# JuliaSmoothOptimizers/Krylov.jl

Measured on NVIDIA H100. Metric: CG iterations/s, higher is better.
Workload: dtype f64

## Files before the change

### krylov.jl_b200/csrc/cg_fused.cu

```cuda
#include "solver_common.h"
#include "spmv_tiles.cuh"

namespace kb {

constexpr int kHist = 64;

template <class T>
struct CgState {
  T gamma, pAp, alpha, beta, pNorm2, rNorm, eps_tol, pad0;
  int iter, itmax, done, linesearch;
  int solved, tired, zero_curvature, inconsistent;
  int npc, not_spd, comm_error, pad2;
  T hist[kHist];
};

static_assert(sizeof(CgState<double>) % 8 == 0 && sizeof(CgState<float>) % 8 == 0, "CgState is copied as 8-byte words");

template <class T>
struct CgPeers {
  HaloMap halo;
  const T* r[kMaxRanks];
  const T* p_old[kMaxRanks];
  const T* mdiag;
  const T* r_halo;
  const T* p_halo_old;
  PushPlan<T> push_p;
};

template <class T>
__device__ __forceinline__ void cg_k1_finalize(CgState<T>* st, T pAp) {
  st->pAp = pAp;
  const T lim = mul_rn(Eps<T>::v, st->pNorm2);
  if (pAp <= lim) {
    if (fabs(pAp) <= lim) { st->zero_curvature = 1; st->inconsistent = !st->linesearch; }
    if (st->linesearch) { st->npc = 1; st->solved = 1; }
    if (st->zero_curvature || st->solved) { st->done = 1; return; }
  }
  st->alpha = div_rn(st->gamma, pAp);
}

template <class T>
__device__ __forceinline__ void cg_k2_finalize(CgState<T>* st, T gamma_next) {
  if (!(gamma_next >= T(0))) { st->not_spd = 1; st->done = 1; return; }
  const T rNorm = sqrt_rn(gamma_next);
  st->rNorm = rNorm;
  const int it1 = st->iter + 1;
  st->hist[it1 % kHist] = rNorm;
  const bool solved = (rNorm <= st->eps_tol) || (add_rn(rNorm, T(1)) <= T(1));
  if (!solved) {
    const T beta = div_rn(gamma_next, st->gamma);
    st->beta = beta;
    st->pNorm2 = add_rn(gamma_next, mul_rn(mul_rn(beta, beta), st->pNorm2));
    st->gamma = gamma_next;
  }
  st->iter = it1;
  st->solved = solved;
  st->tired = it1 >= st->itmax;
  st->done = solved || st->tired;
}

template <class T>
__device__ __forceinline__ bool cg_global_sum(CgState<T>* st, DistComm* dc, T& v) {
  if (dc) {
    v = dist_reduce(dc, v);
    if (dc->error) { st->comm_error = 1; st->done = 1; return false; }
  }
  return true;
}

constexpr int kPlain = 0, kDist = 1, kJacobi = 2, kBlockJac = 3;

template <class T, int MODE>
struct PVal {
  const T* r; const T* p_old; T beta; const CgPeers<T>* peers;
  const T* mdiag;
  __device__ __forceinline__ T operator()(int j) const {
    if (MODE == kDist && j >= peers->halo.nloc) {
      const int h = j - peers->halo.nloc;
      if (peers->r_halo)
        return add_rn(__ldg(&peers->r_halo[h]), mul_rn(beta, __ldg(&peers->p_halo_old[h])));
      const int rk = __ldg(&peers->halo.src_rank[h]), off = __ldg(&peers->halo.src_off[h]);
      return add_rn(__ldg(&peers->r[rk][off]), mul_rn(beta, __ldg(&peers->p_old[rk][off])));
    }
    T z = __ldg(&r[j]);
    if (MODE == kJacobi) z = mul_rn(__ldg(&mdiag[j]), z);
    return add_rn(z, mul_rn(beta, __ldg(&p_old[j])));
  }
};

template <class T> struct RowPre { T pn, po, xr; };

template <class T, int MODE, int MINB, bool XUP>
__global__ void __launch_bounds__(kTileThreads, MINB) cg_k1_tma(Csr<T> A, const T* __restrict__ r, const T* __restrict__ p_old,
                                                          T* __restrict__ p_new, T* __restrict__ Ap, CgState<T>* st,
                                                          T* part, unsigned* ticket, DistComm* dc, CgPeers<T> peers,
                                                          T* __restrict__ x) {
  extern __shared__ __align__(128) unsigned char smem[];
  __shared__ T sm[32];
  if (*(volatile int*)&st->done) return;
  T dacc = T(0);
  bool sent = false;
  const T beta = st->beta, alpha_prev = st->alpha;
  const bool xup = XUP && st->iter > 0;
  const PVal<T, MODE> pval{r, p_old, beta, &peers, peers.mdiag};
  auto row_begin = [&](int row) {
    RowPre<T> q;
    q.po = __ldg(&p_old[row]);
    T z = __ldg(&r[row]);
    if (MODE == kJacobi) z = mul_rn(__ldg(&peers.mdiag[row]), z);
    q.pn = add_rn(z, mul_rn(beta, q.po));
    q.xr = xup ? x[row] : T(0);
    return q;
  };
  spmv_tiles_run<T>(A, smem, pval, row_begin, [&](int row, T acc, RowPre<T> q) {
    p_new[row] = q.pn;
    if (MODE == kDist) sent |= peers.push_p(row, q.pn);
    Ap[row] = acc;
    if (xup) x[row] = add_rn(q.xr, mul_rn(alpha_prev, q.po));
    dacc += q.pn * acc;
  });
  if (MODE == kDist && sent) __threadfence_system();
  T mine[1] = {block_sum(dacc, sm)}, tot[1];
  if (grid_sum_last<T, 1>(mine, part, ticket, sm, tot) && threadIdx.x == 0) {
    if (cg_global_sum(st, MODE == kDist ? dc : nullptr, tot[0])) cg_k1_finalize(st, tot[0]);
  }
}

template <class T, int MODE, bool XUP>
__global__ void __launch_bounds__(kBlock) cg_k1_rows(Csr<T> A, const T* __restrict__ r, const T* __restrict__ p_old,
                                                     T* __restrict__ p_new, T* __restrict__ Ap, CgState<T>* st, T* part,
                                                     unsigned* ticket, DistComm* dc, CgPeers<T> peers, T* __restrict__ x) {
  __shared__ T sm[32];
  if (*(volatile int*)&st->done) return;
  T dacc = T(0);
  bool sent = false;
  const T alpha_prev = st->alpha;
  const bool xup = XUP && st->iter > 0;
  const PVal<T, MODE> pval{r, p_old, st->beta, &peers, peers.mdiag};
  const int stride = gridDim.x * blockDim.x;
  for (int row = blockIdx.x * blockDim.x + threadIdx.x; row < A.n; row += stride) {
    const int kb = A.rowptr[row], ke = A.rowptr[row + 1];
    T acc = T(0);
    for (int k = kb; k < ke; k++) acc = add_rn(acc, mul_rn(A.val[k], pval(A.colind[k])));
    const T pn = pval(row);
    p_new[row] = pn;
    if (MODE == kDist) sent |= peers.push_p(row, pn);
    Ap[row] = acc;
    if (xup) x[row] = add_rn(x[row], mul_rn(alpha_prev, __ldg(&p_old[row])));
    dacc += pn * acc;
  }
  if (MODE == kDist && sent) __threadfence_system();
  T mine[1] = {block_sum(dacc, sm)}, tot[1];
  if (grid_sum_last<T, 1>(mine, part, ticket, sm, tot) && threadIdx.x == 0) {
    if (cg_global_sum(st, MODE == kDist ? dc : nullptr, tot[0])) cg_k1_finalize(st, tot[0]);
  }
}

template <class T, int MODE, bool XK2>
__global__ void __launch_bounds__(kBlock) cg_k2(int n, T* __restrict__ x, T* __restrict__ r, const T* __restrict__ p,
                                                const T* __restrict__ Ap, CgState<T>* st, T* part, unsigned* ticket,
                                                DistComm* dc, const T* __restrict__ mdiag, PushPlan<T> push_r) {
  __shared__ T sm[32];
  if (*(volatile int*)&st->done) return;
  const T alpha = st->alpha, nalpha = -alpha;
  T acc = T(0);
  bool sent = false;
  const int stride = gridDim.x * blockDim.x;
  int i = blockIdx.x * blockDim.x + threadIdx.x;
  for (; i + 3 * stride < n; i += 4 * stride) {
    T xv[4], rv[4], pv[4], av[4];
#pragma unroll
    for (int u = 0; u < 4; u++) {
      const int j = i + u * stride;
      rv[u] = r[j]; av[u] = __ldg(&Ap[j]);
      if (XK2) { xv[u] = x[j]; pv[u] = __ldg(&p[j]); }
    }
#pragma unroll
    for (int u = 0; u < 4; u++) {
      const int j = i + u * stride;
      if (XK2) x[j] = add_rn(xv[u], mul_rn(alpha, pv[u]));
      const T rn = add_rn(rv[u], mul_rn(nalpha, av[u]));
      r[j] = rn;
      if (MODE == kDist) sent |= push_r(j, rn);
      acc += rn * (MODE == kJacobi ? mul_rn(__ldg(&mdiag[j]), rn) : rn);
    }
  }
  for (; i < n; i += stride) {
    const int j = i;
    if (XK2) x[j] = add_rn(x[j], mul_rn(alpha, p[j]));
    const T rn = add_rn(r[j], mul_rn(nalpha, Ap[j]));
    r[j] = rn;
    if (MODE == kDist) sent |= push_r(j, rn);
    acc += rn * (MODE == kJacobi ? mul_rn(__ldg(&mdiag[j]), rn) : rn);
  }
  if (MODE == kDist && sent) __threadfence_system();
  T mine[1] = {block_sum(acc, sm)}, tot[1];
  if (grid_sum_last<T, 1>(mine, part, ticket, sm, tot) && threadIdx.x == 0) {
    if (cg_global_sum(st, dc, tot[0])) cg_k2_finalize(st, tot[0]);
  }
}

struct GridBar { unsigned count, gen, halo_ready, timed_iters; unsigned long long ns_a, ns_b; };

__device__ __forceinline__ unsigned ld_acquire_gpu_u32(const unsigned* p) {
  unsigned v;
  asm volatile("ld.acquire.gpu.global.u32 %0, [%1];" : "=r"(v) : "l"(p) : "memory");
  return v;
}
__device__ __forceinline__ void st_release_gpu_u32(unsigned* p, unsigned v) {
  asm volatile("st.release.gpu.global.u32 [%0], %1;" ::"l"(p), "r"(v) : "memory");
}
__device__ __forceinline__ double ld_sys(const double* p) {
  double v;
  asm volatile("ld.relaxed.sys.global.f64 %0, [%1];" : "=d"(v) : "l"(p) : "memory");
  return v;
}
__device__ __forceinline__ float ld_sys(const float* p) {
  float v;
  asm volatile("ld.relaxed.sys.global.f32 %0, [%1];" : "=f"(v) : "l"(p) : "memory");
  return v;
}

template <class T> struct CgScal { T alpha, beta; int iter, done; };
template <class T>
__device__ __forceinline__ void cg_load_scal(const CgState<T>* st, CgScal<T>* sc) {
  const volatile CgState<T>* v = st;
  const T al = v->alpha, be = v->beta;
  const int it = v->iter, dn = v->done;
  sc->alpha = al; sc->beta = be; sc->iter = it; sc->done = dn;
}

template <class T, class Fin>
__device__ __forceinline__ bool grid_reduce_barrier(GridBar* gb, T v, T* part, T* sm, unsigned* sflag, const CgState<T>* st,
                                                    CgScal<T>* sc, Fin fin) {
  const T mine = block_sum(v, sm);
  if (threadIdx.x == 0) {
    const unsigned g = *(volatile unsigned*)&gb->gen;
    __stcg(&part[blockIdx.x], mine);
    __threadfence();
    const unsigned t = atomicAdd(&gb->count, 1u);
    sflag[0] = (t == gridDim.x - 1);
    sflag[1] = g;
  }
  __syncthreads();
  const bool last = sflag[0] != 0;
  const unsigned g = sflag[1];
  bool ok = true;
  if (last) {
    if (threadIdx.x < 32) {
      __threadfence();
      T acc = T(0);
      for (int i = threadIdx.x; i < (int)gridDim.x; i += 32) acc += __ldcg(&part[i]);
      const T tot = warp_sum(acc);
      fin(tot);
      __syncwarp();
      if (threadIdx.x == 0) {
        cg_load_scal<T>(st, sc);
        gb->count = 0u;
        st_release_gpu_u32(&gb->gen, g + 1u);
      }
    }
  } else if (threadIdx.x == 0) {
    const long long t0 = clock64();
    while (ld_acquire_gpu_u32(&gb->gen) == g) {
      if (clock64() - t0 > 120000000000LL) { sflag[0] = 2; break; }
    }
    cg_load_scal<T>(st, sc);
  }
  __syncthreads();
  if (sflag[0] == 2) ok = false;
  __syncthreads();
  return ok;
}

template <class T>
struct CgPeerTab {
  const T* r[kMaxRanks];
  const T* p[2][kMaxRanks];
};

template <class T>
struct CgPersistArgs {
  T* r; T* P0; T* P1; T* Ap; T* x;
  const T* mdiag;
  T* z;
  const T* mblocks;
  int mbs;
  HaloMap halo;
  const CgPeerTab<T>* tab;
  const int* tile_order;
  int n_interior;
  int max_iters;
  int timed;
  CgState<T>* hsnap;
  unsigned long long* hseq;
  unsigned long long seq;
};

template <class T>
__device__ __forceinline__ void cg_report_to_host(const CgPersistArgs<T>& a, const CgState<T>* st) {
  if (blockIdx.x != 0 || threadIdx.x >= 32 || a.hsnap == nullptr) return;
  const unsigned long long* src = reinterpret_cast<const unsigned long long*>(st);
  unsigned long long* dst = reinterpret_cast<unsigned long long*>(a.hsnap);
  for (int w = threadIdx.x; w < (int)(sizeof(CgState<T>) / 8); w += 32) dst[w] = __ldcg(&src[w]);
  __threadfence_system();
  __syncwarp();
  if (threadIdx.x == 0) { *(volatile unsigned long long*)a.hseq = a.seq; __threadfence_system(); }
}

__device__ __forceinline__ unsigned long long globaltimer_ns() {
  unsigned long long t;
  asm volatile("mov.u64 %0, %globaltimer;" : "=l"(t));
  return t;
}

template <class T, int BS>
__device__ __forceinline__ T cg_phase_b_block(int n, int bs_rt, T nalpha, T* r, const T* Ap, T* z, const T* __restrict__ B, int first, int stride) {
  const int bs = BS ? BS : bs_rt;
  const int nb = (n + bs - 1) / bs;
  T acc = T(0);
  for (int blk = first; blk < nb; blk += stride) {
    const int r0 = blk * bs, rows = min(bs, n - r0);
    T rn[BS ? BS : 8];
#pragma unroll
    for (int i = 0; i < (BS ? BS : 8); i++)
      if (i < rows) { rn[i] = add_rn(r[r0 + i], mul_rn(nalpha, Ap[r0 + i])); r[r0 + i] = rn[i]; }
    const T* Bk = B + (size_t)blk * bs * bs;
#pragma unroll
    for (int i = 0; i < (BS ? BS : 8); i++) {
      if (i < rows) {
        T zi = T(0);
#pragma unroll
        for (int j = 0; j < (BS ? BS : 8); j++)
          if (j < rows) zi = add_rn(zi, mul_rn(__ldg(&Bk[i * bs + j]), rn[j]));
        z[r0 + i] = zi;
        acc += rn[i] * zi;
      }
    }
  }
  return acc;
}

template <class T, int MODE>
__device__ __forceinline__ T cg_phase_b_elems(int n, T nalpha, T* r, const T* Ap, const T* mdiag, int i, int stride) {
  T acc = T(0);
  for (; i + 3 * stride < n; i += 4 * stride) {
    T rv[4], av[4];
#pragma unroll
    for (int u = 0; u < 4; u++) { rv[u] = r[i + u * stride]; av[u] = Ap[i + u * stride]; }
#pragma unroll
    for (int u = 0; u < 4; u++) {
      const int j = i + u * stride;
      const T rn = add_rn(rv[u], mul_rn(nalpha, av[u]));
      r[j] = rn;
      acc += rn * (MODE == kJacobi ? mul_rn(__ldg(&mdiag[j]), rn) : rn);
    }
  }
  for (; i < n; i += stride) {
    const T rn = add_rn(r[i], mul_rn(nalpha, Ap[i]));
    r[i] = rn;
    acc += rn * (MODE == kJacobi ? mul_rn(__ldg(&mdiag[i]), rn) : rn);
  }
  return acc;
}

template <class T>
__device__ __forceinline__ void cg_stage_halo(HaloMap halo, const CgPeerTab<T>* tab, T* r, T* p_old, int pb, int G, int tid, int nthreads) {
  const int nh = halo.nhalo, nloc = halo.nloc;
  const int per = (nh + G - 1) / G;
  const int h0 = (int)blockIdx.x * per, h1 = min(nh, h0 + per);
  for (int h = h0 + tid; h < h1; h += nthreads) {
    const int rk = __ldg(&halo.src_rank[h]), off = __ldg(&halo.src_off[h]);
    const T rv = ld_sys(tab->r[rk] + off);
    const T pv = ld_sys(tab->p[pb][rk] + off);
    __stcg(&r[nloc + h], rv);
    __stcg(&p_old[nloc + h], pv);
  }
}

template <class T, int MODE, class PhaseA>
__device__ __forceinline__ int cg_persist_iterations(int n, const CgPersistArgs<T>& a, CgState<T>* st, T* part, GridBar* gb,
                                                     DistComm* dc, T* sm, unsigned* sflag, CgScal<T>& sc, PhaseA phase_a) {
  const int G = gridDim.x, tid = threadIdx.x, lane = tid & 31;
  int passes = 0;
  for (int k = 0; k < a.max_iters; k++) {
    const int iter = sc.iter;
    const T beta = sc.beta, alpha_prev = sc.alpha;
    T* p_old = (iter & 1) ? a.P1 : a.P0;
    T* p_new = (iter & 1) ? a.P0 : a.P1;
    const bool timing = a.timed && blockIdx.x == 0 && tid == 0;
    unsigned long long t0 = 0, t1 = 0;
    if (timing) t0 = globaltimer_ns();
    const T dacc = phase_a(k, iter, beta, alpha_prev, p_old, p_new);
    passes = k + 1;
    bool ok = grid_reduce_barrier<T>(gb, dacc, part, sm, sflag, st, &sc, [&](T tot) {
      if (MODE == kDist) {
        tot = (T)dist_allreduce_sum_warp<T>(dc, (double)tot);
        if (*(volatile int*)&dc->error) { if (lane == 0) { st->comm_error = 1; st->done = 1; } return; }
      }
      if (lane == 0) cg_k1_finalize(st, tot);
    });
    if (!ok || sc.done) break;
    if (timing) t1 = globaltimer_ns();
    const T nalpha = -sc.alpha;
    const int i = (int)blockIdx.x * kTileThreads + tid, stride = G * kTileThreads;
    T acc;
    if (MODE == kBlockJac) {
      if (a.mbs == 4) acc = cg_phase_b_block<T, 4>(n, 4, nalpha, a.r, a.Ap, a.z, a.mblocks, i, stride);
      else if (a.mbs == 2) acc = cg_phase_b_block<T, 2>(n, 2, nalpha, a.r, a.Ap, a.z, a.mblocks, i, stride);
      else if (a.mbs == 8) acc = cg_phase_b_block<T, 8>(n, 8, nalpha, a.r, a.Ap, a.z, a.mblocks, i, stride);
      else acc = cg_phase_b_block<T, 0>(n, a.mbs, nalpha, a.r, a.Ap, a.z, a.mblocks, i, stride);
    } else {
      acc = cg_phase_b_elems<T, MODE>(n, nalpha, a.r, a.Ap, a.mdiag, i, stride);
    }
    ok = grid_reduce_barrier<T>(gb, acc, part, sm, sflag, st, &sc, [&](T tot) {
      if (MODE == kDist) {
        tot = (T)dist_allreduce_sum_warp<T>(dc, (double)tot);
        if (*(volatile int*)&dc->error) { if (lane == 0) { st->comm_error = 1; st->done = 1; } return; }
      }
      if (lane == 0) {
        cg_k2_finalize(st, tot);
        if (MODE == kDist) gb->halo_ready = 0u;
      }
    });
    if (timing) {
      const unsigned long long t2 = globaltimer_ns();
      gb->ns_a += t1 - t0; gb->ns_b += t2 - t1; gb->timed_iters += 1;
    }
    if (!ok || sc.done) break;
  }
  return passes;
}

template <class T, int MODE, int MINB>
__global__ void __launch_bounds__(kTileThreads, MINB) cg_persist(Csr<T> A, CgPersistArgs<T> a, CgState<T>* st, T* part,
                                                                GridBar* gb, DistComm* dc) {
  extern __shared__ __align__(128) unsigned char smem[];
  __shared__ T sm[32];
  __shared__ unsigned sflag[2];
  __shared__ CgScal<T> sc;
  volatile CgState<T>* vst = st;
  if (vst->done) { cg_report_to_host<T>(a, st); return; }
  if (threadIdx.x == 0) cg_load_scal<T>(st, &sc);
  TilePipe<T> P;
  P.init(A, smem);
  const int G = gridDim.x, tid = threadIdx.x, warp = tid >> 5, lane = tid & 31;
  const int cnt = (A.ntiles - (int)blockIdx.x + G - 1) / G;
  auto tile_at = [&](int j) -> int {
    const int q = blockIdx.x + j * G;
    return MODE == kDist ? __ldg(&a.tile_order[q]) : q;
  };
  const int cnt_int = MODE == kDist ? max(0, min(cnt, (a.n_interior - (int)blockIdx.x + G - 1) / G)) : cnt;
  const unsigned pre = (unsigned)min(P.S, cnt);
  const uint64_t pol = l2_evict_first_policy();
  unsigned ppos = 0, cpos = 0;
  const int passes = cg_persist_iterations<T, MODE>(A.n, a, st, part, gb, dc, sm, sflag, sc,
                                                    [&](int k, int iter, T beta, T alpha_prev, T* p_old, T* p_new) -> T {
    const bool xup = iter > 0;
    T dacc = T(0);
    if (warp == kConsumerWarps) {
      if (lane == 0) {
        const unsigned target = (unsigned)(k + 1) * (unsigned)cnt + (k + 1 < a.max_iters ? pre : 0u);
        tile_issue_until<T>(A, P, ppos, target, cnt, tile_at, pol);
      }
    } else {
      const T* r = MODE == kBlockJac ? a.z : a.r;
      const T* mdiag = a.mdiag;
      auto gather = [&](int j) -> T {
        T z = r[j];
        if (MODE == kJacobi) z = mul_rn(__ldg(&mdiag[j]), z);
        return add_rn(z, mul_rn(beta, p_old[j]));
      };
      auto row_begin = [&](int row) {
        RowPre<T> q;
        q.po = p_old[row];
        T z = r[row];
        if (MODE == kJacobi) z = mul_rn(__ldg(&mdiag[row]), z);
        q.pn = add_rn(z, mul_rn(beta, q.po));
        q.xr = xup ? a.x[row] : T(0);
        return q;
      };
      auto row_done = [&](int row, T acc, RowPre<T> q) {
        p_new[row] = q.pn;
        a.Ap[row] = acc;
        if (xup) a.x[row] = add_rn(q.xr, mul_rn(alpha_prev, q.po));
        dacc += q.pn * acc;
      };
      if (MODE == kDist) {
        cg_stage_halo<T>(a.halo, a.tab, a.r, p_old, iter & 1, G, tid, kTileRows);
        __threadfence();
        __syncwarp();
        if (lane == 0) atomicAdd(&gb->halo_ready, 1u);
        tile_consume_pass<T>(A, P, cpos, 0, cnt_int, tile_at, gather, row_begin, row_done);
        if (cnt_int < cnt) {
          if (lane == 0) { while (ld_acquire_gpu_u32(&gb->halo_ready) < (unsigned)(G * kConsumerWarps)) { } }
          __syncwarp();
          tile_consume_pass<T>(A, P, cpos, cnt_int, cnt, tile_at, gather, row_begin, row_done);
        }
      } else {
        tile_consume_pass<T>(A, P, cpos, 0, cnt, tile_at, gather, row_begin, row_done);
      }
    }
    return dacc;
  });
  if (warp == kConsumerWarps && lane == 0) tile_drain<T>(P, (unsigned)passes * (unsigned)cnt, ppos);
  cg_report_to_host<T>(a, st);
}

template <class T> struct SlotLoads { T r, p, d; };

template <class T, int MODE, int MINB>
__global__ void __launch_bounds__(kTileThreads, 3) cg_persist_dict(CsrDict<T> D, CgPersistArgs<T> a, CgState<T>* st, T* part,
                                                                     GridBar* gb) {
  __shared__ T sm[32];
  __shared__ unsigned sflag[2];
  __shared__ CgScal<T> sc;
  volatile CgState<T>* vst = st;
  if (vst->done) { cg_report_to_host<T>(a, st); return; }
  if (threadIdx.x == 0) cg_load_scal<T>(st, &sc);
  __syncthreads();
  const int G = gridDim.x, tid = threadIdx.x, warp = tid >> 5;
  const int n = D.n, ntiles = (n + kTileRows - 1) / kTileRows;
  const int row0 = (int)blockIdx.x * kTileRows + tid, rstep = G * kTileRows;
  const unsigned m0 = (warp < kConsumerWarps && row0 < n) ? __ldg(&D.mask[row0]) : 0u;
  cg_persist_iterations<T, MODE>(n, a, st, part, gb, nullptr, sm, sflag, sc,
                                 [&](int, int iter, T beta, T alpha_prev, const T* p_old, T* p_new) -> T {
    const bool xup = iter > 0;
    T dacc = T(0);
    if (warp < kConsumerWarps) {
      const T* r = a.r;
      const T* mdiag = a.mdiag;
      auto load = [&](int j) -> SlotLoads<T> {
        return SlotLoads<T>{r[j], p_old[j], MODE == kJacobi ? __ldg(&mdiag[j]) : T(0)};
      };
      auto value = [&](const SlotLoads<T>& l) -> T {
        const T z = MODE == kJacobi ? mul_rn(l.d, l.r) : l.r;
        return add_rn(z, mul_rn(beta, l.p));
      };
      unsigned m = m0;
      SlotLoads<T> nxt{};
      T xnxt = T(0);
      if (row0 < n) { nxt = load(row0); xnxt = xup ? a.x[row0] : T(0); }
      for (int t = blockIdx.x, row = row0; t < ntiles; t += G, row += rstep) {
        const unsigned mnext = (t + G < ntiles && row + rstep < n) ? __ldg(&D.mask[row + rstep]) : 0u;
        if (row < n) {
          const SlotLoads<T> here = nxt;
          const T xr = xnxt;
          if (t + G < ntiles && row + rstep < n) { nxt = load(row + rstep); xnxt = xup ? a.x[row + rstep] : T(0); }
          const T po = here.p;
          const T pn = value(here);
          const T acc = dict_row_sum<T>(D, row, m, load, value);
          p_new[row] = pn;
          a.Ap[row] = acc;
          if (xup) a.x[row] = add_rn(xr, mul_rn(alpha_prev, po));
          dacc += pn * acc;
        }
        m = mnext;
      }
    }
    return dacc;
  });
  cg_report_to_host<T>(a, st);
}

template <class T>
__global__ void push_ranges_kernel(const T* __restrict__ v, PushPlan<T> plan) {
  const int stride = gridDim.x * blockDim.x, tid = blockIdx.x * blockDim.x + threadIdx.x;
  for (int q = 0; q < plan.nranges; q++)
    for (int d = tid; d < plan.rg[q].count; d += stride) plan.dst[q][plan.rg[q].slot + d] = v[plan.rg[q].start + d];
  __threadfence_system();
}

template <class T> void cg_dist_push_r(Workspace<T>& ws) {
  if (ws.dist.world <= 1 || ws.dist.npush <= 0) return;
  PushPlan<T> plan;
  memset(&plan, 0, sizeof(plan));
  plan.nranges = ws.dist.npush;
  for (int q = 0; q < ws.dist.npush; q++) { plan.rg[q] = ws.dist.push[q]; plan.dst[q] = ws.dist.halo_buf_peer[plan.rg[q].peer]; }
  push_ranges_kernel<T><<<sm_count(), kBlock, 0, ws.ctx.stream>>>(ws.r, plan);
  KB_CUDA(cudaGetLastError());
  ws.ctx.launches++;
}

constexpr size_t kOffGridBar = 1024, kOffPeerTab = 2048, kOffHostSeq = 3072;

template <class T> void fused_block_alloc(Workspace<T>& ws) {
  KB_CUDA(cudaMalloc(&ws.fused_state, kFusedBlockBytes));
  KB_CUDA(cudaMemset(ws.fused_state, 0, kFusedBlockBytes));
  KB_CUDA(cudaHostAlloc(&ws.fused_host, kFusedBlockBytes, cudaHostAllocPortable | cudaHostAllocMapped));
  memset(ws.fused_host, 0, kFusedBlockBytes);
}

template <class T> void cg_fused_prepare(Workspace<T>& ws) {
  static_assert(sizeof(CgState<T>) <= kOffGridBar && sizeof(CgPeerTab<T>) <= kFusedBlockBytes - kOffPeerTab, "block layout");
  if (!ws.p2) ws.p2 = dev_alloc<T>((size_t)ws.n);
  for (int i = 0; i < 2; i++)
    if (!ws.fused_ev[i]) KB_CUDA(cudaEventCreateWithFlags(&ws.fused_ev[i], cudaEventDisableTiming));
}

template <class T>
__global__ void tile_halo_flags_kernel(Csr<T> A, int nloc, int* flags) {
  const int warp = (blockIdx.x * blockDim.x + threadIdx.x) >> 5, lane = threadIdx.x & 31;
  const int nw = (gridDim.x * blockDim.x) >> 5;
  for (int t = warp; t < A.ntiles; t += nw) {
    const int k0 = A.rowptr[t * kTileRows], k1 = A.rowptr[min(t * kTileRows + kTileRows, A.n)];
    bool any = false;
    for (int k = k0 + lane; k < k1; k += 32) any |= A.colind[k] >= nloc;
    any = __any_sync(0xffffffffu, any);
    if (lane == 0) flags[t] = any ? 1 : 0;
  }
}

template <class T> void cg_dist_tile_order(Workspace<T>& ws, const Csr<T>& A) {
  if (ws.dist.tile_order && ws.dist.tile_order_for == (const void*)A.rowptr && ws.dist.tile_order_n == A.ntiles) return;
  Ctx& c = ws.ctx;
  if (ws.dist.tile_order) { cudaFree(ws.dist.tile_order); ws.dist.tile_order = nullptr; }
  const int nt = A.ntiles;
  KB_CUDA(cudaMalloc((void**)&ws.dist.tile_order, sizeof(int) * (size_t)(nt > 0 ? nt : 1)));
  if (nt > 0) {
    tile_halo_flags_kernel<T><<<sm_count() * 4, 256, 0, c.stream>>>(A, ws.n, ws.dist.tile_order);
    KB_CUDA(cudaGetLastError());
    std::vector<int> fl(nt), ord;
    KB_CUDA(cudaMemcpyAsync(fl.data(), ws.dist.tile_order, sizeof(int) * nt, cudaMemcpyDeviceToHost, c.stream));
    c.sync();
    ord.reserve(nt);
    for (int t = 0; t < nt; t++) if (!fl[t]) ord.push_back(t);
    ws.dist.tile_order_interior = (int)ord.size();
    for (int t = 0; t < nt; t++) if (fl[t]) ord.push_back((int)((unsigned)t | 0x80000000u));
    KB_CUDA(cudaMemcpyAsync(ws.dist.tile_order, ord.data(), sizeof(int) * nt, cudaMemcpyHostToDevice, c.stream));
    c.sync();
  }
  ws.dist.tile_order_for = (const void*)A.rowptr;
  ws.dist.tile_order_n = nt;
}

template <class T>
CgFusedPlan<T> cg_fused_plan(const Workspace<T>& ws, const LinOp<T>& A, const LinOp<T>& M, const SolveOpts& o) {
  CgFusedPlan<T> pl;
  const bool dist = ws.dist.world > 1;
  const bool jac = M.kind == LinOp<T>::DIAG && !o.ldiv, bjac = M.kind == LinOp<T>::BDIAG && !o.ldiv;
  if (!o.fused || A.kind != LinOp<T>::CSR || o.radius != 0 || !(M.is_identity() || jac || bjac) || (dist && !M.is_identity()))
    return pl;
  const Csr<T>& C = *A.csr;
  const int n = ws.n;
  pl.single_step = (o.callback != nullptr) || (o.timemax < 1e300) || o.verbose > 0;
  const char* exu = getenv("KB200_XUP");
  pl.xup = !pl.single_step && !(exu && atoi(exu) == 0);
  pl.persist = C.tma_ok && pl.xup && o.persist != 0;
  if (bjac && !pl.persist) return pl;
  pl.fused = true;
  pl.A = &C;
  pl.mdiag = jac ? M.diag : nullptr;
  pl.mblocks = bjac ? M.blocks : nullptr;
  pl.mbs = bjac ? M.bs : 0;
  pl.batch = pl.single_step ? 1 : (o.batch > 0 ? std::min(o.batch, kHist / 2) : 32);
  if (pl.persist) {
    if (bjac) pl.kp = cg_persist<T, kBlockJac, 2>;
    else if (C.ctas_per_sm >= 3) pl.kp = dist ? cg_persist<T, kDist, 3> : (jac ? cg_persist<T, kJacobi, 3> : cg_persist<T, kPlain, 3>);
    else pl.kp = dist ? cg_persist<T, kDist, 2> : (jac ? cg_persist<T, kJacobi, 2> : cg_persist<T, kPlain, 2>);
    ensure_dyn_smem((const void*)pl.kp, 220 * 1024);
    int occ = 0;
    KB_CUDA(cudaOccupancyMaxActiveBlocksPerMultiprocessor(&occ, pl.kp, kTileThreads, C.smem_bytes));
    if (occ < 1) throw std::runtime_error("cg_persist does not fit on an SM with the planned shared-memory ring");
    pl.pgrid = std::min(std::min(occ, C.ctas_per_sm) * sm_count(), std::max(1, C.ntiles));
    const CsrDict<T>* dict = A.dict;
    if (dict && dict->npairs > 0 && dict->n == n && !dist && !bjac) {
      const typename CgFusedPlan<T>::KdFn kd =
          C.ctas_per_sm >= 3 ? (jac ? cg_persist_dict<T, kJacobi, 3> : cg_persist_dict<T, kPlain, 3>)
                             : (jac ? cg_persist_dict<T, kJacobi, 2> : cg_persist_dict<T, kPlain, 2>);
      int occd = 0;
      KB_CUDA(cudaOccupancyMaxActiveBlocksPerMultiprocessor(&occd, kd, kTileThreads, 0));
      if (occd * sm_count() >= pl.pgrid) { pl.kd = kd; pl.dict = dict; }
    }
    return pl;
  }
  const bool xup = pl.xup;
  if (C.tma_ok) {
    if (dist) pl.k1 = xup ? cg_k1_tma<T, kDist, 3, true> : cg_k1_tma<T, kDist, 3, false>;
    else if (jac) pl.k1 = xup ? cg_k1_tma<T, kJacobi, 3, true> : cg_k1_tma<T, kJacobi, 3, false>;
    else if (C.ctas_per_sm >= 4) pl.k1 = xup ? cg_k1_tma<T, kPlain, 4, true> : cg_k1_tma<T, kPlain, 4, false>;
    else if (C.ctas_per_sm == 3) pl.k1 = xup ? cg_k1_tma<T, kPlain, 3, true> : cg_k1_tma<T, kPlain, 3, false>;
    else pl.k1 = xup ? cg_k1_tma<T, kPlain, 1, true> : cg_k1_tma<T, kPlain, 1, false>;
    ensure_dyn_smem((const void*)pl.k1, 220 * 1024);
    int occ = 0;
    KB_CUDA(cudaOccupancyMaxActiveBlocksPerMultiprocessor(&occ, pl.k1, kTileThreads, C.smem_bytes));
    if (occ < 1) throw std::runtime_error("cg_k1_tma does not fit on an SM with the planned shared-memory ring");
    pl.k1_grid = std::min(std::min(occ, C.ctas_per_sm) * sm_count(), std::max(1, C.ntiles));
    pl.k1_block = kTileThreads;
    pl.k1_smem = C.smem_bytes;
  } else {
    if (dist) pl.k1 = xup ? cg_k1_rows<T, kDist, true> : cg_k1_rows<T, kDist, false>;
    else if (jac) pl.k1 = xup ? cg_k1_rows<T, kJacobi, true> : cg_k1_rows<T, kJacobi, false>;
    else pl.k1 = xup ? cg_k1_rows<T, kPlain, true> : cg_k1_rows<T, kPlain, false>;
    pl.k1_grid = stream_grid(n, 1, 8);
    pl.k1_block = kBlock;
    pl.k1_smem = 0;
  }
  if (dist) pl.k2 = xup ? cg_k2<T, kDist, false> : cg_k2<T, kDist, true>;
  else if (jac) pl.k2 = xup ? cg_k2<T, kJacobi, false> : cg_k2<T, kJacobi, true>;
  else pl.k2 = xup ? cg_k2<T, kPlain, false> : cg_k2<T, kPlain, true>;
  pl.k2_grid = stream_grid(n, 4, 8);
  return pl;
}

template <class T>
CgFusedExit cg_fused_loop(Workspace<T>& ws, const CgFusedPlan<T>& pl, const SolveOpts& o, T gamma0, T eps_tol, int itmax,
                          double start_time) {
  Ctx& c = ws.ctx;
  const int n = ws.n;
  typedef CgState<T> St;
  const bool dist = ws.dist.world > 1;
  const Csr<T>& A = *pl.A;
  cg_fused_prepare<T>(ws);
  St* dst = (St*)ws.fused_state;
// ... 218 lines not shown
```

### krylov.jl_b200/csrc/spmv_tiles.cuh

```cuda
#pragma once
#include "common.cuh"
#include "kb_internal.h"

namespace kb {

constexpr int kConsumerWarps = kTileRows / 32;
constexpr int kTileThreads = kTileRows + 32;
constexpr int kGatherDepth = 8;
#ifndef KB_CLAMP_GATHER
#define KB_CLAMP_GATHER 1
#endif

__device__ __forceinline__ uint32_t smem_u32(const void* p) { return (uint32_t)__cvta_generic_to_shared(p); }
__device__ __forceinline__ void mbar_init(uint64_t* bar, unsigned count) {
  asm volatile("mbarrier.init.shared::cta.b64 [%0], %1;" ::"r"(smem_u32(bar)), "r"(count));
}
__device__ __forceinline__ void mbar_expect_tx(uint64_t* bar, unsigned bytes) {
  asm volatile("mbarrier.arrive.expect_tx.shared::cta.b64 _, [%0], %1;" ::"r"(smem_u32(bar)), "r"(bytes) : "memory");
}
__device__ __forceinline__ void mbar_arrive(uint64_t* bar) {
  asm volatile("mbarrier.arrive.shared::cta.b64 _, [%0];" ::"r"(smem_u32(bar)) : "memory");
}
__device__ __forceinline__ void mbar_wait(uint64_t* bar, unsigned parity) {
  unsigned ok;
// ... 130 lines not shown
  }
  __syncthreads();

  if (warp == kConsumerWarps) {
    if (lane == 0) tile_producer<T>(A, L, S, ring, full, empty);
  } else {
    int it = 0;
    for (int t = blockIdx.x; t < A.ntiles; t += gridDim.x, it++) {
      const int row = t * kTileRows + tid;
      auto pre = row_begin(row < A.n ? row : 0);
      const int s = it % S;
      mbar_wait(&full[s], (it / S) & 1);
      const unsigned char* st = ring + (size_t)s * L.stage_bytes();
      const int* rp = reinterpret_cast<const int*>(st);
      const T* vs = reinterpret_cast<const T*>(st + L.rp_bytes());
      const int* cs = reinterpret_cast<const int*>(st + L.rp_bytes() + L.val_bytes());
      if (row < A.n) {
        const int k0 = rp[0];
        const T* vrow = vs - (k0 & ~(VA - 1));
        const int* crow = cs - (k0 & ~3);
        const int kb = rp[tid], ke = rp[tid + 1];
        T acc = T(0);
        for (int k = kb; k < ke; k += kGatherDepth) {
          T xv[kGatherDepth], av[kGatherDepth];
#if KB_CLAMP_GATHER
#pragma unroll
          for (int u = 0; u < kGatherDepth; u++) {
            const int kk = min(k + u, ke - 1);
            av[u] = vrow[kk];
            xv[u] = gather(crow[kk]);
          }
          asm volatile("" ::: "memory");
#pragma unroll
          for (int u = 0; u < kGatherDepth; u++) {
            const T nx = add_rn(acc, mul_rn(av[u], xv[u]));
            acc = (k + u < ke) ? nx : acc;
          }
#else
#pragma unroll
          for (int u = 0; u < kGatherDepth; u++) {
            if (k + u < ke) { av[u] = vrow[k + u]; xv[u] = gather(crow[k + u]); }
          }
#pragma unroll
          for (int u = 0; u < kGatherDepth; u++) {
            if (k + u < ke) acc = add_rn(acc, mul_rn(av[u], xv[u]));
          }
#endif
        }
        row_done(row, acc, pre);
      }
      __syncwarp();
      if (lane == 0) mbar_arrive(&empty[s]);
    }
  }
}


template <class T>
struct TilePipe {
  TileLayout<T> L;
  int S;
  uint64_t* full;
  uint64_t* empty;
  unsigned char* ring;
  __device__ __forceinline__ void init(const Csr<T>& A, unsigned char* smem) {
    L = TileLayout<T>{A.tile_cap};
    S = A.stages;
    full = reinterpret_cast<uint64_t*>(smem);
    empty = full + S;
    ring = smem + 128;
    if (threadIdx.x == 0) {
      for (int s = 0; s < S; s++) { mbar_init(&full[s], 1); mbar_init(&empty[s], kConsumerWarps); }
      asm volatile("fence.mbarrier_init.release.cluster;" ::: "memory");
    }
    __syncthreads();
  }
};

template <class T, class TileAt>
__device__ __forceinline__ void tile_issue_until(const Csr<T>& A, const TilePipe<T>& P, unsigned& pos, unsigned target, int cnt,
                                                 TileAt tile_at, uint64_t pol) {
  constexpr int VA = 16 / sizeof(T);
  if (pos >= target) return;
  int t = tile_at((int)(pos % (unsigned)cnt)) & 0x7fffffff;
  int k0 = __ldg(&A.rowptr[t * kTileRows]), k1 = __ldg(&A.rowptr[min(t * kTileRows + kTileRows, A.n)]);
  for (; pos < target; pos++) {
    int tn = 0, nk0 = 0, nk1 = 0;
    if (pos + 1 < target) {
      tn = tile_at((int)((pos + 1) % (unsigned)cnt)) & 0x7fffffff;
      nk0 = __ldg(&A.rowptr[tn * kTileRows]); nk1 = __ldg(&A.rowptr[min(tn * kTileRows + kTileRows, A.n)]);
    }
    const int s = (int)(pos % (unsigned)P.S);
    mbar_wait(&P.empty[s], ((pos / (unsigned)P.S) & 1) ^ 1);
    unsigned char* st = P.ring + (size_t)s * P.L.stage_bytes();
    const int k0v = k0 & ~(VA - 1), k1v = (k1 + VA - 1) & ~(VA - 1);
    const int k0c = k0 & ~3, k1c = (k1 + 3) & ~3;
    const unsigned rp_b = (kTileRows + 4) * sizeof(int);
    const unsigned v_b = (unsigned)(k1v - k0v) * sizeof(T);
    const unsigned c_b = (unsigned)(k1c - k0c) * sizeof(int);
    mbar_expect_tx(&P.full[s], rp_b + v_b + c_b);
    tma_load_1d(st, A.rowptr + t * kTileRows, rp_b, &P.full[s], pol);
    if (v_b) tma_load_1d(st + P.L.rp_bytes(), A.val + k0v, v_b, &P.full[s], pol);
    if (c_b) tma_load_1d(st + P.L.rp_bytes() + P.L.val_bytes(), A.colind + k0c, c_b, &P.full[s], pol);
    t = tn; k0 = nk0; k1 = nk1;
  }
}

template <class T>
__device__ __forceinline__ void tile_drain(const TilePipe<T>& P, unsigned consumed, unsigned pos) {
  for (unsigned q = consumed; q < pos; q++) mbar_wait(&P.full[q % (unsigned)P.S], (q / (unsigned)P.S) & 1);
}

template <class T, class TileAt, class Gather, class RowBegin, class RowDone>
__device__ __forceinline__ void tile_consume_pass(const Csr<T>& A, const TilePipe<T>& P, unsigned& cpos, int j0, int j1, TileAt tile_at,
                                                  Gather gather, RowBegin row_begin, RowDone row_done) {
  constexpr int VA = 16 / sizeof(T);
  const int tid = threadIdx.x, lane = tid & 31;
  for (int j = j0; j < j1; j++, cpos++) {
    const int t = tile_at(j) & 0x7fffffff;
    const int row = t * kTileRows + tid;
    auto pre = row_begin(row < A.n ? row : 0);
    const int s = (int)(cpos % (unsigned)P.S);
    mbar_wait(&P.full[s], (cpos / (unsigned)P.S) & 1);
    const unsigned char* st = P.ring + (size_t)s * P.L.stage_bytes();
    const int* rp = reinterpret_cast<const int*>(st);
    const T* vs = reinterpret_cast<const T*>(st + P.L.rp_bytes());
    const int* cs = reinterpret_cast<const int*>(st + P.L.rp_bytes() + P.L.val_bytes());
    if (row < A.n) {
      const int k0 = rp[0];
      const T* vrow = vs - (k0 & ~(VA - 1));
      const int* crow = cs - (k0 & ~3);
      const int kb = rp[tid], ke = rp[tid + 1];
      T acc = T(0);
      for (int k = kb; k < ke; k += kGatherDepth) {
        T xv[kGatherDepth], av[kGatherDepth];
#pragma unroll
        for (int u = 0; u < kGatherDepth; u++) xv[u] = gather(crow[min(k + u, ke - 1)]);
        asm volatile("" ::: "memory");
#pragma unroll
        for (int u = 0; u < kGatherDepth; u++) av[u] = vrow[min(k + u, ke - 1)];
#pragma unroll
        for (int u = 0; u < kGatherDepth; u++) {
          const T nx = add_rn(acc, mul_rn(av[u], xv[u]));
          acc = (k + u < ke) ? nx : acc;
        }
      }
      row_done(row, acc, pre);
    }
    __syncwarp();
    if (lane == 0) mbar_arrive(&P.empty[s]);
  }
}

template <class T, class Load, class Value>
__device__ __forceinline__ T dict_row_sum(const CsrDict<T>& D, int row, unsigned m, Load load, Value value) {
  decltype(load(0)) lv[kDictSlots];
#pragma unroll
  for (int u = 0; u < kDictSlots; u++) lv[u] = load(((m >> u) & 1u) ? row + D.off[u] : row);
  asm volatile("" ::: "memory");
  T acc = T(0);
#pragma unroll
  for (int u = 0; u < kDictSlots; u++) {
    const T nx = add_rn(acc, mul_rn(D.val[u], value(lv[u])));
    acc = ((m >> u) & 1u) ? nx : acc;
  }
  return acc;
}

}
```

### profiles/ab_cg_dict.py

```python
import argparse
import filecmp
import json
import os
import statistics
import subprocess
import sys
import tempfile

ROOT = os.path.dirname(os.path.dirname(os.path.abspath(__file__)))


def gpu_info():
    q = subprocess.run(["nvidia-smi", "--query-gpu=name,power.limit,clocks.max.sm", "--format=csv,noheader"],
                       capture_output=True, text=True).stdout.strip().splitlines()
    return q[0] if q else "unknown"


def bench(lib, extra):
    env = dict(os.environ)
    env.pop("KB200_LIB", None)
    if lib:
        env["KB200_LIB"] = lib
    r = subprocess.run([sys.executable, os.path.join(ROOT, "bench.py"), "--gpus", "1", "--steps", "5", "--warmup", "3"] + extra,
                       env=env, capture_output=True, text=True, cwd=ROOT)
    lines = [l for l in r.stdout.splitlines() if l.startswith("{")]
    if r.returncode != 0 or not lines:
        raise SystemExit(f"bench.py failed ({lib or 'current'}): {r.stderr[-3000:]}")
    return json.loads(lines[-1])


def summary(recs):
    med = lambda f: statistics.median(f(r) for r in recs)
    out = dict(values=[r["value"] for r in recs], value=med(lambda r: r["value"]),
               cfg5_values=[r.get("cfg5", {}).get("value") for r in recs],
               cfg5_value=med(lambda r: r.get("cfg5", {}).get("value") or 0.0),
               e2e=med(lambda r: r["e2e"]["value"]),
               extra={e["config"]: statistics.median(x["value"] for r in recs for x in r.get("extra", []) if x.get("config") == e["config"])
                      for e in recs[0].get("extra", []) if "config" in e},
               kernels=recs[0]["roofline"]["kernels"], frac_csr_model=med(lambda r: r["roofline"]["frac"]))
    return out


def main():
    ap = argparse.ArgumentParser()
    ap.add_argument("parent_lib")
    ap.add_argument("--runs", type=int, default=3)
    ap.add_argument("--out", default=None)
    args = ap.parse_args()
    libs = {"parent": os.path.abspath(args.parent_lib), "encoded": None}
    recs = {k: [] for k in libs}
    with tempfile.TemporaryDirectory() as tmp:
        for i in range(args.runs):
            for name, lib in libs.items():
                extra = ["--dump-outputs", os.path.join(tmp, name)] if i == 0 else ["--no-cpu"]
                recs[name].append(bench(lib, extra))
                print(name, i, recs[name][-1]["value"], flush=True)
        same = {f: filecmp.cmp(os.path.join(tmp, "parent", f), os.path.join(tmp, "encoded", f), shallow=False)
                for f in sorted(os.listdir(os.path.join(tmp, "parent")))}
    line = dict(gpu=gpu_info(), runs=args.runs, dumps_identical=same,
                parity_max_rel_dev={k: v[0].get("parity", {}).get("max_rel_dev") for k, v in recs.items()},
                **{k: summary(v) for k, v in recs.items()})
    cfg = recs["encoded"][0]["config"]
    n, iters = cfg["n"], cfg["iters_per_step"]
    b_dict = n + 9 * n * 8 + 96
    enc = line["encoded"]
    enc["bytes_per_iteration_dict"] = b_dict
    enc["GBs_dict"] = b_dict * enc["value"] / 1e9
    k = enc["kernels"]
    for ph, b in (("phase_a", n + 6 * n * 8), ("phase_b", 3 * n * 8)):
        ms = k[ph]["ms"]
        k[ph]["bytes_dict"] = b
        k[ph]["GBs_dict"] = b / (ms * 1e-3) / 1e9 if ms else None
    line["speedup"] = enc["value"] / line["parent"]["value"]
    line["cfg5_speedup"] = enc["cfg5_value"] / line["parent"]["cfg5_value"] if line["parent"]["cfg5_value"] else None
    txt = json.dumps(line)
    print(txt)
    if args.out:
        with open(args.out, "a") as f:
            f.write(txt + "\n")


if __name__ == "__main__":
    main()
```

Baseline: 3742.

## Recompute Ap in phase B and defer x updates to alternate iterations

In the dictionary-encoded CG kernel, phase A no longer stores Ap. Phase B recomputes A*p from p_new, with three rows unrolled per thread, so the Ap write and read are replaced by reads of p that are likely cached. The x update is also split by tile-parity: each tile updates x only every other iteration and applies two steps at once using a stored alpha_prev. A fix-up at termination applies the pending step. Together these cut global memory traffic per iteration at the cost of redoing the SpMV arithmetic and more complex termination bookkeeping.

Result: slower. 3702, median of 6 (-1.1%).

```diff
diff --git a/krylov.jl_b200/csrc/cg_fused.cu b/krylov.jl_b200/csrc/cg_fused.cu
--- a/krylov.jl_b200/csrc/cg_fused.cu
+++ b/krylov.jl_b200/csrc/cg_fused.cu
@@ -7,7 +7,8 @@
 
 template <class T>
 struct CgState {
-  T gamma, pAp, alpha, beta, pNorm2, rNorm, eps_tol, pad0;
+  T gamma, pAp, alpha, beta, pNorm2, rNorm, eps_tol;
+  T alpha_prev;
   int iter, itmax, done, linesearch;
   int solved, tired, zero_curvature, inconsistent;
   int npc, not_spd, comm_error, pad2;
@@ -36,6 +37,7 @@
     if (st->linesearch) { st->npc = 1; st->solved = 1; }
     if (st->zero_curvature || st->solved) { st->done = 1; return; }
   }
+  st->alpha_prev = st->alpha;
   st->alpha = div_rn(st->gamma, pAp);
 }
 
@@ -221,13 +223,13 @@
   return v;
 }
 
-template <class T> struct CgScal { T alpha, beta; int iter, done; };
+template <class T> struct CgScal { T alpha, beta, alpha_prev; int iter, done; };
 template <class T>
 __device__ __forceinline__ void cg_load_scal(const CgState<T>* st, CgScal<T>* sc) {
   const volatile CgState<T>* v = st;
-  const T al = v->alpha, be = v->beta;
+  const T al = v->alpha, be = v->beta, ap = v->alpha_prev;
   const int it = v->iter, dn = v->done;
-  sc->alpha = al; sc->beta = be; sc->iter = it; sc->done = dn;
+  sc->alpha = al; sc->beta = be; sc->alpha_prev = ap; sc->iter = it; sc->done = dn;
 }
 
 template <class T, class Fin>
@@ -378,10 +380,11 @@
   }
 }
 
-template <class T, int MODE, class PhaseA>
-__device__ __forceinline__ int cg_persist_iterations(int n, const CgPersistArgs<T>& a, CgState<T>* st, T* part, GridBar* gb,
-                                                     DistComm* dc, T* sm, unsigned* sflag, CgScal<T>& sc, PhaseA phase_a) {
-  const int G = gridDim.x, tid = threadIdx.x, lane = tid & 31;
+template <class T, int MODE, class PhaseA, class PhaseB>
+__device__ __forceinline__ int cg_persist_iterations(const CgPersistArgs<T>& a, CgState<T>* st, T* part, GridBar* gb,
+                                                     DistComm* dc, T* sm, unsigned* sflag, CgScal<T>& sc, PhaseA phase_a,
+                                                     PhaseB phase_b) {
+  const int tid = threadIdx.x, lane = tid & 31;
   int passes = 0;
   for (int k = 0; k < a.max_iters; k++) {
     const int iter = sc.iter;
@@ -402,17 +405,7 @@
     });
     if (!ok || sc.done) break;
     if (timing) t1 = globaltimer_ns();
-    const T nalpha = -sc.alpha;
-    const int i = (int)blockIdx.x * kTileThreads + tid, stride = G * kTileThreads;
-    T acc;
-    if (MODE == kBlockJac) {
-      if (a.mbs == 4) acc = cg_phase_b_block<T, 4>(n, 4, nalpha, a.r, a.Ap, a.z, a.mblocks, i, stride);
-      else if (a.mbs == 2) acc = cg_phase_b_block<T, 2>(n, 2, nalpha, a.r, a.Ap, a.z, a.mblocks, i, stride);
-      else if (a.mbs == 8) acc = cg_phase_b_block<T, 8>(n, 8, nalpha, a.r, a.Ap, a.z, a.mblocks, i, stride);
-      else acc = cg_phase_b_block<T, 0>(n, a.mbs, nalpha, a.r, a.Ap, a.z, a.mblocks, i, stride);
-    } else {
-      acc = cg_phase_b_elems<T, MODE>(n, nalpha, a.r, a.Ap, a.mdiag, i, stride);
-    }
+    const T acc = phase_b(-sc.alpha, p_new);
     ok = grid_reduce_barrier<T>(gb, acc, part, sm, sflag, st, &sc, [&](T tot) {
       if (MODE == kDist) {
         tot = (T)dist_allreduce_sum_warp<T>(dc, (double)tot);
@@ -454,7 +447,7 @@
   const unsigned pre = (unsigned)min(P.S, cnt);
   const uint64_t pol = l2_evict_first_policy();
   unsigned ppos = 0, cpos = 0;
-  const int passes = cg_persist_iterations<T, MODE>(A.n, a, st, part, gb, dc, sm, sflag, sc,
+  const int passes = cg_persist_iterations<T, MODE>(a, st, part, gb, dc, sm, sflag, sc,
                                                     [&](int k, int iter, T beta, T alpha_prev, T* p_old, T* p_new) -> T {
     const bool xup = iter > 0;
     T dacc = T(0);
@@ -502,6 +495,15 @@
       }
     }
     return dacc;
+  }, [&](T nalpha, const T*) -> T {
+    const int n = A.n, i = (int)blockIdx.x * kTileThreads + tid, stride = G * kTileThreads;
+    if (MODE == kBlockJac) {
+      if (a.mbs == 4) return cg_phase_b_block<T, 4>(n, 4, nalpha, a.r, a.Ap, a.z, a.mblocks, i, stride);
+      if (a.mbs == 2) return cg_phase_b_block<T, 2>(n, 2, nalpha, a.r, a.Ap, a.z, a.mblocks, i, stride);
+      if (a.mbs == 8) return cg_phase_b_block<T, 8>(n, 8, nalpha, a.r, a.Ap, a.z, a.mblocks, i, stride);
+      return cg_phase_b_block<T, 0>(n, a.mbs, nalpha, a.r, a.Ap, a.z, a.mblocks, i, stride);
+    }
+    return cg_phase_b_elems<T, MODE>(n, nalpha, a.r, a.Ap, a.mdiag, i, stride);
   });
   if (warp == kConsumerWarps && lane == 0) tile_drain<T>(P, (unsigned)passes * (unsigned)cnt, ppos);
   cg_report_to_host<T>(a, st);
@@ -522,10 +524,14 @@
   const int G = gridDim.x, tid = threadIdx.x, warp = tid >> 5;
   const int n = D.n, ntiles = (n + kTileRows - 1) / kTileRows;
   const int row0 = (int)blockIdx.x * kTileRows + tid, rstep = G * kTileRows;
+  const int i0 = (int)blockIdx.x * kTileThreads + tid, istep = G * kTileThreads;
+  const int iter0 = sc.iter;
   const unsigned m0 = (warp < kConsumerWarps && row0 < n) ? __ldg(&D.mask[row0]) : 0u;
-  cg_persist_iterations<T, MODE>(n, a, st, part, gb, nullptr, sm, sflag, sc,
-                                 [&](int, int iter, T beta, T alpha_prev, const T* p_old, T* p_new) -> T {
-    const bool xup = iter > 0;
+  const int passes = cg_persist_iterations<T, MODE>(a, st, part, gb, nullptr, sm, sflag, sc,
+                                                    [&](int, int iter, T beta, T alpha_prev, const T* p_old, T* p_new) -> T {
+    auto xup = [&](int t) { return iter >= 1 && !((t ^ iter) & 1); };
+    const bool two = iter >= 2;
+    const T alpha_pp = sc.alpha_prev;
     T dacc = T(0);
     if (warp < kConsumerWarps) {
       const T* r = a.r;
@@ -539,27 +545,75 @@
       };
       unsigned m = m0;
       SlotLoads<T> nxt{};
-      T xnxt = T(0);
-      if (row0 < n) { nxt = load(row0); xnxt = xup ? a.x[row0] : T(0); }
+      T xnxt = T(0), qnxt = T(0);
+      if (row0 < n) {
+        nxt = load(row0);
+        if (xup(blockIdx.x)) { xnxt = a.x[row0]; if (two) qnxt = p_new[row0]; }
+      }
       for (int t = blockIdx.x, row = row0; t < ntiles; t += G, row += rstep) {
         const unsigned mnext = (t + G < ntiles && row + rstep < n) ? __ldg(&D.mask[row + rstep]) : 0u;
         if (row < n) {
           const SlotLoads<T> here = nxt;
-          const T xr = xnxt;
-          if (t + G < ntiles && row + rstep < n) { nxt = load(row + rstep); xnxt = xup ? a.x[row + rstep] : T(0); }
+          const T xr = xnxt, pq = qnxt;
+          if (t + G < ntiles && row + rstep < n) {
+            nxt = load(row + rstep);
+            if (xup(t + G)) { xnxt = a.x[row + rstep]; if (two) qnxt = p_new[row + rstep]; }
+          }
           const T po = here.p;
           const T pn = value(here);
           const T acc = dict_row_sum<T>(D, row, m, load, value);
           p_new[row] = pn;
-          a.Ap[row] = acc;
-          if (xup) a.x[row] = add_rn(xr, mul_rn(alpha_prev, po));
+          if (xup(t)) a.x[row] = add_rn(two ? add_rn(xr, mul_rn(alpha_pp, pq)) : xr, mul_rn(alpha_prev, po));
           dacc += pn * acc;
         }
         m = mnext;
       }
     }
     return dacc;
+  }, [&](T nalpha, const T* p_new) -> T {
+    auto load = [&](int j) -> T { return p_new[j]; };
+    auto value = [](T v) -> T { return v; };
+    auto fetch = [&](int j, unsigned& m, T& rv, T& d) {
+      m = 0u; rv = T(0); d = T(0);
+      if (j < n) { m = __ldg(&D.mask[j]); rv = a.r[j]; if (MODE == kJacobi) d = __ldg(&a.mdiag[j]); }
+    };
+    constexpr int R = 3;
+    T acc = T(0);
+    unsigned mc[R];
+    T rc[R], dc[R];
+#pragma unroll
+    for (int q = 0; q < R; q++) fetch(i0 + q * istep, mc[q], rc[q], dc[q]);
+    for (int i = i0; i < n; i += R * istep) {
+      unsigned mn[R];
+      T rnx[R], dn[R];
+      int rows[R];
+#pragma unroll
+      for (int q = 0; q < R; q++) {
+        fetch(i + (R + q) * istep, mn[q], rnx[q], dn[q]);
+        rows[q] = i + q * istep < n ? i + q * istep : i;
+      }
+      T ap[R];
+      dict_rows_sum<T, R>(D, rows, mc, load, value, ap);
+#pragma unroll
+      for (int q = 0; q < R; q++) {
+        const int j = i + q * istep;
+        if (j < n) {
+          const T rn = add_rn(rc[q], mul_rn(nalpha, ap[q]));
+          a.r[j] = rn;
+          acc += rn * (MODE == kJacobi ? mul_rn(dc[q], rn) : rn);
+        }
+        mc[q] = mn[q]; rc[q] = rnx[q]; dc[q] = dn[q];
+      }
+    }
+    return acc;
   });
+  const int k = iter0 + passes - 1;
+  if (sc.done && k >= 1) {
+    const T al = (vst->zero_curvature || vst->npc) ? vst->alpha : vst->alpha_prev;
+    const T* p = (k & 1) ? a.P1 : a.P0;
+    for (int i = i0; i < n; i += istep)
+      if ((i / kTileRows ^ k) & 1) a.x[i] = add_rn(a.x[i], mul_rn(al, p[i]));
+  }
   cg_report_to_host<T>(a, st);
 }
 
diff --git a/krylov.jl_b200/csrc/spmv_tiles.cuh b/krylov.jl_b200/csrc/spmv_tiles.cuh
--- a/krylov.jl_b200/csrc/spmv_tiles.cuh
+++ b/krylov.jl_b200/csrc/spmv_tiles.cuh
@@ -306,18 +306,30 @@
   }
 }
 
+template <class T, int R, class Load, class Value>
+__device__ __forceinline__ void dict_rows_sum(const CsrDict<T>& D, const int* row, const unsigned* m, Load load, Value value,
+                                              T* acc) {
+  decltype(load(0)) lv[R][kDictSlots];
+#pragma unroll
+  for (int q = 0; q < R; q++)
+#pragma unroll
+    for (int u = 0; u < kDictSlots; u++) lv[q][u] = load(((m[q] >> u) & 1u) ? row[q] + D.off[u] : row[q]);
+  asm volatile("" ::: "memory");
+#pragma unroll
+  for (int q = 0; q < R; q++) {
+    acc[q] = T(0);
+#pragma unroll
+    for (int u = 0; u < kDictSlots; u++) {
+      const T nx = add_rn(acc[q], mul_rn(D.val[u], value(lv[q][u])));
+      acc[q] = ((m[q] >> u) & 1u) ? nx : acc[q];
+    }
+  }
+}
+
 template <class T, class Load, class Value>
 __device__ __forceinline__ T dict_row_sum(const CsrDict<T>& D, int row, unsigned m, Load load, Value value) {
-  decltype(load(0)) lv[kDictSlots];
-#pragma unroll
-  for (int u = 0; u < kDictSlots; u++) lv[u] = load(((m >> u) & 1u) ? row + D.off[u] : row);
-  asm volatile("" ::: "memory");
-  T acc = T(0);
-#pragma unroll
-  for (int u = 0; u < kDictSlots; u++) {
-    const T nx = add_rn(acc, mul_rn(D.val[u], value(lv[u])));
-    acc = ((m >> u) & 1u) ? nx : acc;
-  }
+  T acc;
+  dict_rows_sum<T, 1>(D, &row, &m, load, value, &acc);
   return acc;
 }
 
diff --git a/profiles/ab_cg_dict.py b/profiles/ab_cg_dict.py
--- a/profiles/ab_cg_dict.py
+++ b/profiles/ab_cg_dict.py
@@ -62,12 +62,12 @@
                 **{k: summary(v) for k, v in recs.items()})
     cfg = recs["encoded"][0]["config"]
     n, iters = cfg["n"], cfg["iters_per_step"]
-    b_dict = n + 9 * n * 8 + 96
+    b_dict = 2 * n + 60 * n + 96
     enc = line["encoded"]
     enc["bytes_per_iteration_dict"] = b_dict
     enc["GBs_dict"] = b_dict * enc["value"] / 1e9
     k = enc["kernels"]
-    for ph, b in (("phase_a", n + 6 * n * 8), ("phase_b", 3 * n * 8)):
+    for ph, b in (("phase_a", n + 36 * n), ("phase_b", n + 24 * n)):
         ms = k[ph]["ms"]
         k[ph]["bytes_dict"] = b
         k[ph]["GBs_dict"] = b / (ms * 1e-3) / 1e9 if ms else None
```
